# wangjie212/ManiSDP-matlab

Hardware: AMD Instinct MI355X
Metric: tCG Hess-vec prods/sec (n,p), G81 MaxCut (higher is better)
Workload: dtype f64; 1 GPU; Gset G81 MaxCut, ManiSDP_onlyunitdiag RTR call, n=20000, p=32; n=20000, p=32, nnz_C=92644, TR_maxiter=40, TR_maxinner=100, parallelism=rows1

## Files before the change

manisdp-matlab_amd/csrc/msdp_pipe.h:

```cpp
#pragma once
#include <type_traits>
#include "msdp_psync.h"

template <class F>
__device__ __forceinline__ bool psync8(unsigned long long* slots, unsigned gen, int G, double (&v)[8], double* sh8, double* shb8, int* err,
                                       int bid, int backoff, unsigned long long* tr, F on_ready) {
    const int lane = threadIdx.x & 63, w = threadIdx.x >> 6;
    {
        const bool h8 = (lane & 8) != 0;
        double a[4], b[2], x;
#pragma unroll
        for (int k = 0; k < 4; ++k) a[k] = msdp_swap_add<32>(v[k], v[4 + k]);
#pragma unroll
        for (int k = 0; k < 2; ++k) b[k] = msdp_swap_add<16>(a[k], a[2 + k]);
        x = (h8 ? b[1] : b[0]) + msdp_dpp<0x128>(h8 ? b[0] : b[1]);
        x += msdp_dpp<MSDP_DPP_XOR1>(x); x += msdp_dpp<MSDP_DPP_XOR2>(x); x += msdp_dpp<MSDP_DPP_HALF_MIRROR>(x);
        if ((lane & 7) == 0) sh8[(lane >> 3) * PWAVES + w] = x;
    }
    if (tr && threadIdx.x == 0) tr[4] = __builtin_readcyclecounter();
    asm volatile("s_waitcnt vmcnt(0)" ::: "memory");
    __syncthreads();
    if (tr && threadIdx.x == 0) tr[2] = __builtin_readcyclecounter();
    {
        unsigned long long* gbase = slots + (size_t)(gen % PSYNC_GEN) * PSYNC_REP * PSYNC_NV * MSDP_MAX_GRID;
        if (w == 0) {
            const int rep = lane / PSYNC_NV, vi = lane % PSYNC_NV;
            double s = 0.0;
            for (int i = 0; i < PWAVES; ++i) s += sh8[vi * PWAVES + i];
            asm volatile("s_waitcnt vmcnt(0)" ::: "memory");
            __hip_atomic_store(gbase + ((size_t)rep * PSYNC_NV + vi) * MSDP_MAX_GRID + bid,
                               (unsigned long long)__double_as_longlong(s), __ATOMIC_RELAXED, __HIP_MEMORY_SCOPE_AGENT);
        }
        const unsigned long long* p0 = gbase + ((size_t)(bid & (PSYNC_REP - 1)) * PSYNC_NV + w) * MSDP_MAX_GRID + lane;
        double r0;
        int spins = 0;
        bool fail = false;
        const int first = ((backoff >> 16) & 0xff) ? ((backoff >> 16) & 0xff) : 27;
        for (int q = 0; q < first; ++q) __builtin_amdgcn_s_sleep(1);
        if (tr && threadIdx.x == 0) tr[3] = __builtin_readcyclecounter();
        for (;;) {
            unsigned long long b0[4];
            asm volatile(
                "global_load_dwordx2 %0, %4, off sc1\n\t"
                "global_load_dwordx2 %1, %4, off offset:512 sc1\n\t"
                "global_load_dwordx2 %2, %4, off offset:1024 sc1\n\t"
                "global_load_dwordx2 %3, %4, off offset:1536 sc1\n\t"
                "s_waitcnt vmcnt(0)"
                : "=&v"(b0[0]), "=&v"(b0[1]), "=&v"(b0[2]), "=&v"(b0[3])
                : "v"(p0)
                : "memory");
            bool ok = true;
            double t0 = 0.0;
#pragma unroll
            for (int q = 0; q < 4; ++q) {
                if (lane + 64 * q < G) {
                    ok = ok && b0[q] != PSYNC_SENT;
                    t0 += __longlong_as_double((long long)b0[q]);
                }
            }
            r0 = t0;
            if (__builtin_amdgcn_ballot_w64(!ok) == 0ULL) break;
            ++spins;
            if (spins > PSYNC_SPIN_LIMIT ||
                ((spins & 1023) == 0 && __hip_atomic_load(err, __ATOMIC_RELAXED, __HIP_MEMORY_SCOPE_AGENT))) { fail = true; break; }
            for (int q = 0; q < ((backoff >> 8) & 0xff); ++q) __builtin_amdgcn_s_sleep(1);
        }
        if (tr && threadIdx.x == 0) tr[7] = (__builtin_readcyclecounter() << 4) + (unsigned long long)(spins < 15 ? spins : 15);
        if (!fail) on_ready();
        r0 = msdp_wave_sum(r0);
        if (lane == 0) {
            shb8[w] = r0; shb8[8 + w] = fail ? 1.0 : 0.0;
            if (fail) __hip_atomic_store(err, 1, __ATOMIC_RELAXED, __HIP_MEMORY_SCOPE_AGENT);
        }
        if (w == 0)
            __hip_atomic_store(slots + (size_t)((gen + PSYNC_GEN - 1) % PSYNC_GEN) * PSYNC_REP * PSYNC_NV * MSDP_MAX_GRID +
                                   (size_t)lane * MSDP_MAX_GRID + bid,
                               PSYNC_SENT, __ATOMIC_RELAXED, __HIP_MEMORY_SCOPE_AGENT);
    }
    asm volatile("s_waitcnt lgkmcnt(0)\n\ts_barrier" ::: "memory");
    double bad = 0.0;
#pragma unroll
    for (int i = 0; i < 8; ++i) { v[i] = msdp_readlane(shb8[i], 0); bad += msdp_readlane(shb8[8 + i], 0); }
    return bad == 0.0;
}

typedef unsigned long long v2ul __attribute__((ext_vector_type(2)));
template <class F>
__device__ __forceinline__ bool psync8_lines(unsigned long long* slots, unsigned gen, int G, double (&v)[8], double* sh8, double* shp, double* shb8,
                                             int* err, int bid, int backoff, unsigned long long* tr, F on_ready) {
    const int lane = threadIdx.x & 63, w = threadIdx.x >> 6;
    {
        const bool h8 = (lane & 8) != 0;
        double a[4], b[2], x;
#pragma unroll
        for (int k = 0; k < 4; ++k) a[k] = msdp_swap_add<32>(v[k], v[4 + k]);
#pragma unroll
        for (int k = 0; k < 2; ++k) b[k] = msdp_swap_add<16>(a[k], a[2 + k]);
        x = (h8 ? b[1] : b[0]) + msdp_dpp_all<0x128>(h8 ? b[0] : b[1]);
        x += msdp_dpp_all<MSDP_DPP_XOR1>(x); x += msdp_dpp_all<MSDP_DPP_XOR2>(x); x += msdp_dpp_all<MSDP_DPP_HALF_MIRROR>(x);
        if ((lane & 7) == 0) sh8[(lane >> 3) * PWAVES + w] = x;
    }
    if (tr && threadIdx.x == 0) tr[4] = __builtin_readcyclecounter();
    asm volatile("s_waitcnt vmcnt(0)" ::: "memory");
    __syncthreads();
    if (tr && threadIdx.x == 0) tr[2] = __builtin_readcyclecounter();
    unsigned long long* gbase = slots + (size_t)(gen % PSYNC_GEN) * PSYNC_REP * PSYNC_NV * MSDP_MAX_GRID;
    if (w == 0) {
        const int rep = lane >> 3, vi = lane & 7;
        double s = 0.0;
        for (int i = 0; i < PWAVES; ++i) s += sh8[vi * PWAVES + i];
        asm volatile("s_waitcnt vmcnt(0)" ::: "memory");
        __hip_atomic_store(gbase + (size_t)rep * PSYNC_NV * MSDP_MAX_GRID + (size_t)bid * 8 + vi,
                           (unsigned long long)__double_as_longlong(s), __ATOMIC_RELAXED, __HIP_MEMORY_SCOPE_AGENT);
    }
    const unsigned long long* p0 = gbase + (size_t)(bid & (PSYNC_REP - 1)) * PSYNC_NV * MSDP_MAX_GRID + (size_t)(32 * w + (lane >> 2)) * 8 + 2 * (lane & 3);
    const bool in0 = 32 * w + (lane >> 2) < G, in1 = 32 * w + 16 + (lane >> 2) < G;
    double t0 = 0.0, t1 = 0.0;
    int spins = 0;
    bool fail = false;
    const int first = ((backoff >> 16) & 0xff) ? ((backoff >> 16) & 0xff) : (backoff & 0xff);
    for (int q = 0; q < first; ++q) __builtin_amdgcn_s_sleep(1);
    if (tr && threadIdx.x == 0) tr[3] = __builtin_readcyclecounter();
    if (__builtin_amdgcn_ballot_w64(in0) != 0ULL) {
        for (;;) {
            v2ul a0, a1;
            asm volatile(
                "global_load_dwordx4 %0, %2, off sc1\n\t"
                "global_load_dwordx4 %1, %2, off offset:1024 sc1\n\t"
                "s_waitcnt vmcnt(0)"
                : "=&v"(a0), "=&v"(a1)
                : "v"(p0)
                : "memory");
            bool ok = true;
            t0 = 0.0; t1 = 0.0;
            if (in0) { ok = a0.x != PSYNC_SENT && a0.y != PSYNC_SENT; t0 = __longlong_as_double((long long)a0.x); t1 = __longlong_as_double((long long)a0.y); }
            if (in1) { ok = ok && a1.x != PSYNC_SENT && a1.y != PSYNC_SENT; t0 += __longlong_as_double((long long)a1.x); t1 += __longlong_as_double((long long)a1.y); }
            if (__builtin_amdgcn_ballot_w64(!ok) == 0ULL) break;
            ++spins;
            if (spins > PSYNC_SPIN_LIMIT ||
                ((spins & 1023) == 0 && __hip_atomic_load(err, __ATOMIC_RELAXED, __HIP_MEMORY_SCOPE_AGENT))) { fail = true; break; }
            for (int q = 0; q < ((backoff >> 8) & 0xff); ++q) __builtin_amdgcn_s_sleep(1);
        }
    }
    if (tr && threadIdx.x == 0) tr[7] = (__builtin_readcyclecounter() << 4) + (unsigned long long)(spins < 15 ? spins : 15);
    t0 += msdp_dpp_all<0x124>(t0); t1 += msdp_dpp_all<0x124>(t1);
    t0 += msdp_dpp_all<0x128>(t0); t1 += msdp_dpp_all<0x128>(t1);
    t0 = msdp_rowpair_sum<16>(t0); t1 = msdp_rowpair_sum<16>(t1);
    t0 = msdp_rowpair_sum<32>(t0); t1 = msdp_rowpair_sum<32>(t1);
    if (lane < 4) { shp[w * 8 + 2 * lane] = t0; shp[w * 8 + 2 * lane + 1] = t1; }
    if (lane == 0) {
        shb8[8 + w] = fail ? 1.0 : 0.0;
        if (fail) __hip_atomic_store(err, 1, __ATOMIC_RELAXED, __HIP_MEMORY_SCOPE_AGENT);
    }
    asm volatile("s_waitcnt lgkmcnt(0)\n\ts_barrier" ::: "memory");
    on_ready();
    if (w == 0)
        __hip_atomic_store(slots + (size_t)((gen + PSYNC_GEN - 1) % PSYNC_GEN) * PSYNC_REP * PSYNC_NV * MSDP_MAX_GRID +
                               (size_t)(lane >> 3) * PSYNC_NV * MSDP_MAX_GRID + (size_t)bid * 8 + (lane & 7),
                           PSYNC_SENT, __ATOMIC_RELAXED, __HIP_MEMORY_SCOPE_AGENT);
    double s = 0.0;
#pragma unroll
    for (int k = 0; k < PWAVES; ++k) s += shp[k * 8 + (lane & 7)];
    const double fl = shb8[8 + (lane & 7)];
#pragma unroll
    for (int i = 0; i < 8; ++i) v[i] = msdp_readlane(s, i);
    return __builtin_amdgcn_ballot_w64(fl != 0.0) == 0ULL;
}

__device__ __forceinline__ bool pbar8_lines(unsigned long long* slots, unsigned gen, int G, double* shb8, int* err, int bid, int backoff) {
    const int lane = threadIdx.x & 63, w = threadIdx.x >> 6;
    asm volatile("s_waitcnt vmcnt(0)" ::: "memory");
    __syncthreads();
    unsigned long long* gbase = slots + (size_t)(gen % PSYNC_GEN) * PSYNC_REP * PSYNC_NV * MSDP_MAX_GRID;
    if (w == 0) {
        asm volatile("s_waitcnt vmcnt(0)" ::: "memory");
        __hip_atomic_store(gbase + (size_t)(lane >> 3) * PSYNC_NV * MSDP_MAX_GRID + (size_t)bid * 8 + (lane & 7), 0ULL, __ATOMIC_RELAXED, __HIP_MEMORY_SCOPE_AGENT);
    }
    const unsigned long long* p0 = gbase + (size_t)(bid & (PSYNC_REP - 1)) * PSYNC_NV * MSDP_MAX_GRID + (size_t)(32 * w + (lane >> 2)) * 8 + 2 * (lane & 3);
    const bool in0 = 32 * w + (lane >> 2) < G, in1 = 32 * w + 16 + (lane >> 2) < G;
    int spins = 0;
    bool fail = false;
    const int first = ((backoff >> 16) & 0xff) ? ((backoff >> 16) & 0xff) : (backoff & 0xff);
    for (int q = 0; q < first; ++q) __builtin_amdgcn_s_sleep(1);
    if (__builtin_amdgcn_ballot_w64(in0) != 0ULL) {
        for (;;) {
            v2ul a0, a1;
            asm volatile(
                "global_load_dwordx4 %0, %2, off sc1\n\t"
                "global_load_dwordx4 %1, %2, off offset:1024 sc1\n\t"
                "s_waitcnt vmcnt(0)"
                : "=&v"(a0), "=&v"(a1)
                : "v"(p0)
                : "memory");
            bool ok = true;
            if (in0) ok = a0.x != PSYNC_SENT && a0.y != PSYNC_SENT;
            if (in1) ok = ok && a1.x != PSYNC_SENT && a1.y != PSYNC_SENT;
            if (__builtin_amdgcn_ballot_w64(!ok) == 0ULL) break;
            ++spins;
            if (spins > PSYNC_SPIN_LIMIT ||
                ((spins & 1023) == 0 && __hip_atomic_load(err, __ATOMIC_RELAXED, __HIP_MEMORY_SCOPE_AGENT))) { fail = true; break; }
            for (int q = 0; q < ((backoff >> 8) & 0xff); ++q) __builtin_amdgcn_s_sleep(1);
        }
    }
    if (lane == 0) {
        shb8[8 + w] = fail ? 1.0 : 0.0;
        if (fail) __hip_atomic_store(err, 1, __ATOMIC_RELAXED, __HIP_MEMORY_SCOPE_AGENT);
    }
    asm volatile("s_waitcnt lgkmcnt(0)\n\ts_barrier" ::: "memory");
    if (w == 0)
        __hip_atomic_store(slots + (size_t)((gen + PSYNC_GEN - 1) % PSYNC_GEN) * PSYNC_REP * PSYNC_NV * MSDP_MAX_GRID +
                               (size_t)(lane >> 3) * PSYNC_NV * MSDP_MAX_GRID + (size_t)bid * 8 + (lane & 7),
                           PSYNC_SENT, __ATOMIC_RELAXED, __HIP_MEMORY_SCOPE_AGENT);
    const double fl = shb8[8 + (lane & 7)];
    return __builtin_amdgcn_ballot_w64(fl != 0.0) == 0ULL;
}

template <class F>
__device__ __forceinline__ bool psync2_8(unsigned long long* blk, unsigned long long* const* peers, int N, int me, int ri, unsigned gen, int G,
                                         double (&v)[8], double* sh8, double* shb8, int* err, int bid, int backoff, F on_ready) {
    const int lane = threadIdx.x & 63, w = threadIdx.x >> 6;
    {
        const bool h8 = (lane & 8) != 0;
        double a[4], b[2], x;
#pragma unroll
        for (int k = 0; k < 4; ++k) a[k] = msdp_swap_add<32>(v[k], v[4 + k]);
#pragma unroll
        for (int k = 0; k < 2; ++k) b[k] = msdp_swap_add<16>(a[k], a[2 + k]);
        x = (h8 ? b[1] : b[0]) + msdp_dpp<0x128>(h8 ? b[0] : b[1]);
        x += msdp_dpp<MSDP_DPP_XOR1>(x); x += msdp_dpp<MSDP_DPP_XOR2>(x); x += msdp_dpp<MSDP_DPP_HALF_MIRROR>(x);
        if ((lane & 7) == 0) sh8[(lane >> 3) * PWAVES + w] = x;
    }
    asm volatile("s_waitcnt vmcnt(0)" ::: "memory");
    __syncthreads();
    unsigned long long* ls = blk + (size_t)ri * XR2_REGION;
    unsigned long long* ml = ls + PSYNC_REGION;
    unsigned long long* gbase = ls + (size_t)(gen % PSYNC_GEN) * PSYNC_REP * PSYNC_NV * MSDP_MAX_GRID;
    if (w == 0 && lane < 8) {
        double s = 0.0;
        for (int i = 0; i < PWAVES; ++i) s += sh8[lane * PWAVES + i];
        asm volatile("s_waitcnt vmcnt(0)" ::: "memory");
        __hip_atomic_store(gbase + (size_t)lane * MSDP_MAX_GRID + bid, (unsigned long long)__double_as_longlong(s), __ATOMIC_RELAXED, __HIP_MEMORY_SCOPE_AGENT);
    }
    bool fail = false;
    if (bid == 0) {
        const unsigned long long* p0 = gbase + (size_t)w * MSDP_MAX_GRID + lane;
        double r0 = 0.0;
        int spins = 0;
        for (;;) {
            unsigned long long b0[4];
            asm volatile(
                "global_load_dwordx2 %0, %4, off sc1\n\t"
                "global_load_dwordx2 %1, %4, off offset:512 sc1\n\t"
                "global_load_dwordx2 %2, %4, off offset:1024 sc1\n\t"
                "global_load_dwordx2 %3, %4, off offset:1536 sc1\n\t"
                "s_waitcnt vmcnt(0)"
                : "=&v"(b0[0]), "=&v"(b0[1]), "=&v"(b0[2]), "=&v"(b0[3])
                : "v"(p0)
                : "memory");
            bool ok = true;
            double t0 = 0.0;
#pragma unroll
            for (int q = 0; q < 4; ++q) {
                if (lane + 64 * q < G) {
                    ok = ok && b0[q] != PSYNC_SENT;
                    t0 += __longlong_as_double((long long)b0[q]);
                }
            }
            r0 = t0;
            if (__builtin_amdgcn_ballot_w64(!ok) == 0ULL) break;
            ++spins;
            if (spins > PSYNC_SPIN_LIMIT || ((spins & 1023) == 0 && __hip_atomic_load(err, __ATOMIC_RELAXED, __HIP_MEMORY_SCOPE_AGENT))) { fail = true; break; }
        }
        r0 = msdp_wave_sum(r0);
        if (!fail && lane < N)
            __hip_atomic_store(peers[lane] + (size_t)ri * XR2_REGION + PSYNC_REGION + ((size_t)(gen % PSYNC_GEN) * 8 + me) * 8 + w,
                               (unsigned long long)__double_as_longlong(r0), __ATOMIC_RELAXED, __HIP_MEMORY_SCOPE_SYSTEM);
        if (fail) xr2_fail(blk, peers, N, err);
        if (w > 0 && lane == 0) shb8[8 + w] = fail ? 1.0 : 0.0;
    }
    if (w == 0) {
        const unsigned long long* p = ml + (size_t)(gen % PSYNC_GEN) * 64 + lane;
        const bool need = (lane >> 3) < N;
        const int first = bid == 0 ? 0 : (((backoff >> 16) & 0xff) ? ((backoff >> 16) & 0xff) : (backoff & 0xff));
        for (int q = 0; q < first; ++q) __builtin_amdgcn_s_sleep(1);
        unsigned long long x = 0ULL;
        int spins = 0;
        for (;;) {
            x = ld_u64_sys(p);
            if (__builtin_amdgcn_ballot_w64(need && x == PSYNC_SENT) == 0ULL) break;
            ++spins;
            if (spins > PSYNC_SPIN_LIMIT || ((spins & 1023) == 0 && __hip_atomic_load(err, __ATOMIC_RELAXED, __HIP_MEMORY_SCOPE_AGENT))) { fail = true; break; }
            for (int q = 0; q < ((backoff >> 8) & 0xff); ++q) __builtin_amdgcn_s_sleep(1);
        }
        double t = need ? __longlong_as_double((long long)x) : 0.0;
        t += msdp_dpp<0x128>(t);
        t = msdp_rowpair_sum<16>(t);
        t = msdp_rowpair_sum<32>(t);
        if (lane < 8) { shb8[lane] = t; if (bid != 0 && lane > 0) shb8[8 + lane] = 0.0; }
        if (lane == 0) shb8[8] = fail ? 1.0 : 0.0;
        if (fail) xr2_fail(blk, peers, N, err);
        if (lane < PSYNC_NV)
            __hip_atomic_store(ls + (size_t)((gen + PSYNC_GEN - 1) % PSYNC_GEN) * PSYNC_REP * PSYNC_NV * MSDP_MAX_GRID + (size_t)lane * MSDP_MAX_GRID + bid,
                               PSYNC_SENT, __ATOMIC_RELAXED, __HIP_MEMORY_SCOPE_AGENT);
        if (bid == 0)
            __hip_atomic_store(ml + (size_t)((gen + PSYNC_GEN - 1) % PSYNC_GEN) * 64 + lane, PSYNC_SENT, __ATOMIC_RELAXED, __HIP_MEMORY_SCOPE_AGENT);
    }
    __syncthreads();
    on_ready();
    double bad = 0.0;
#pragma unroll
    for (int i = 0; i < 8; ++i) { v[i] = msdp_readlane(shb8[i], 0); bad += msdp_readlane(shb8[8 + i], 0); }
    return bad == 0.0;
}

#ifndef MSDP_PIPE_LINES
#define MSDP_PIPE_LINES 1
#endif
#if MSDP_PIPE_LINES
#define PSYNC8(slots, gen, G, v, sh8, shb8, err, bid, backoff, tr, f) psync8_lines(slots, gen, G, v, sh8, shp, shb8, err, bid, backoff, tr, f)
#else
#define PSYNC8(slots, gen, G, v, sh8, shb8, err, bid, backoff, tr, f) psync8(slots, gen, G, v, sh8, shb8, err, bid, backoff, tr, f)
#endif
template <int LPR, int EW, int R, bool TRACE, bool FUSE, int XRM = 0, int EP = 1>
__device__ __forceinline__ void tcg_pipe_body(const Dev& d, unsigned long long* slots, int* err, const int bx) {
    constexpr bool XR = XRM != 0, XTWO = XRM == 2;
    constexpr bool CSR = EW == 0;
    static_assert(!XR || (!FUSE && !TRACE), "cross-rank instances: per-iteration launches");
    static_assert(R <= 5, "pipelined trip: every vector in registers");
    static_assert(CSR ? (EP == 64 / LPR && !XR && !TRACE) : EP == 1, "CSR rows: one row per wave, one rank");
    static_assert(PSYNC_NV == 8 && PSYNC_REP * PSYNC_NV == 64, "psync8 posts one slot per lane of wave 0");
    constexpr bool BOFF = !(EW == 8 && LPR == 16), ROWB_INV = !XTWO, UMASK = !(FUSE && LPR == 16);
    extern __shared__ double lds[];
    __shared__ double sh8[8 * PWAVES];
    __shared__ double shp[8 * PWAVES];
    __shared__ double shb8[16];
    constexpr int RPW = 64 / (LPR * EP);
    constexpr int RSTEP = PWAVES * RPW;
    constexpr int ROWS = R * RSTEP;
    double2* Ys = reinterpret_cast<double2*>(lds);
    double2* Gs = Ys + R * PB;
    double* eGs = reinterpret_cast<double*>(Gs + R * PB);
    double* vs = eGs + ROWS;
    int* cs = reinterpret_cast<int*>(vs + EW * ROWS);
    int* ls = cs + EW * ROWS;
    double2* HQs = reinterpret_cast<double2*>(ls + EW * ROWS);
    unsigned long long* pds = reinterpret_cast<unsigned long long*>(HQs + 2 * R * PB);
    double2* YPs = HQs + 2 * R * PB;
    double2* GPs = YPs + R * PB;
    double* EGPs = reinterpret_cast<double*>(GPs + R * PB);

    const Ctl* c = d.ctl;
    const bool lead = bx == 0 && threadIdx.x == 0;
    const int k_tr = c->k;
    if (c->done) {
        if (lead) {
            frame_store(&d.F[0], c->gg, c->gg, 0.0, 0.0, 0.0, sqrt(c->gg), 0.0, 0.0, 0, 0, 5, 0, 0, 1);
            d.ctl->tcg_running = 0;
            msdp_publish(d, k_tr, 0, 0);
        }
        return;
    }
    if (lead && !FUSE) msdp_publish(d, k_tr, 0, 1);
    const int bid = (XR && !XTWO) ? d.xr_gid0 + bx : bx;
    const int GS = (XR && !XTWO) ? d.xr_gtot : d.G;
    const int xri = k_tr & 1;
    __shared__ unsigned long long* shpeer[XTWO ? 8 : 1];
    if (XTWO) {
        if (threadIdx.x < 8) shpeer[threadIdx.x] = threadIdx.x < d.xr2_n ? d.xr2_peers[threadIdx.x] : d.xr2_blk;
        psync2_reset_other(d.xr2_blk, xri ^ 1, bid, GS);
        asm volatile("s_waitcnt vmcnt(0)" ::: "memory");
    } else if (XR) {
        unsigned long long* other = slots + (size_t)(xri ^ 1) * PSYNC_REGION;
        slots += (size_t)xri * PSYNC_REGION;
        psync_reset_other(other, bid, GS);
        asm volatile("s_waitcnt vmcnt(0)" ::: "memory");
    } else if (!FUSE) psync_reset_other(slots + PSYNC_REGION, bid, GS);
    int lo, hi;
    msdp_chunk_rows(d.n_loc, d.G, lo, hi, 0, bx);
    const int lane = threadIdx.x & 63, wave = threadIdx.x >> 6;
    const int sub = lane & (LPR - 1), rsub = lane / (LPR * EP);
    const int epi = (lane / LPR) & (EP - 1);
    const bool colok_g = 2 * sub < d.ld;
    const bool colok = colok_g && epi == 0;
    int cur = c->cur;
    const bool bench = c->bench_mode != 0;
    double Delta = c->Delta;
    const double kappa = c->kappa, theta = c->theta;
    const int mininner = c->mininner, maxinner = c->maxinner;
    double gg = c->gg;
    double fx = c->fx;
    int k_it = c->k;
    const double Delta_bar = c->Delta_bar, rho_prime = c->rho_prime, rho_reg_opt = c->rho_reg, tolgradnorm = c->tolgradnorm;
    const int maxiter = c->maxiter;
    int n_acc = c->accepted, n_rej = c->rejected, n_hv = c->hessvecs, n_ce = c->cost_evals;
    const double* __restrict__ Yl = cur ? d.Y[1] : d.Y[0];
    const double* __restrict__ gl = cur ? d.Gr[1] : d.Gr[0];
    const double* __restrict__ eGl = cur ? d.eG[1] : d.eG[0];
    const int slot0 = wave * RPW + rsub;
#define SLOT(r) ((r) * RSTEP + slot0)
#define ROW(r) (lo + SLOT(r))
#define ROK(r) (ROW(r) < hi)
#define OK(r) (ROK(r) && colok)
    const unsigned rowb0 = ((unsigned)(lo + slot0) * (unsigned)d.ld + 2u * (unsigned)sub) * 8u;
#define ROWB(r) (ROWB_INV ? (rowb0 + (unsigned)((r) * RSTEP) * (unsigned)d.ld * 8u) : (((unsigned)ROW(r) * gld + 2 * sub) * 8u))
    const int refresh = c->pipe_refresh;
    const int backoff = (c->psync_backoff & 0xff00ffff) | ((((c->psync_backoff >> 16) & 0xff) ? ((c->psync_backoff >> 16) & 0xff) : (c->psync8_backoff & 0xff)) << 16);
    const double2 zz = make_double2(0.0, 0.0);
    const unsigned gld = (unsigned)d.ld;
    constexpr bool LOC = !CSR && R * EW <= 15;
    constexpr bool MULTI = LOC && !(FUSE && LPR >= 16);
    double2 eta[R], rr[R], md[R], hmd[R], cmd[R], ctr[R];
#pragma unroll
    for (int r = 0; r < R; ++r) {
        const bool rok = ROK(r);
        const int rc = rok ? ROW(r) : lo;
        const int64_t o = (int64_t)rc * d.ld + (colok ? 2 * sub : 0);
        double2 y = ld2(Yl + o), g = ld2(gl + o);
        if (!OK(r)) { y = zz; g = zz; }
        Ys[r * PB + threadIdx.x] = y; Gs[r * PB + threadIdx.x] = g;
        eta[r] = zz; rr[r] = g; md[r] = g; hmd[r] = zz; cmd[r] = zz; ctr[r] = zz;
    }
#pragma unroll 1
    for (int r = 0; r < (CSR ? 0 : R); ++r) {
        const bool rok = ROK(r);
        const int rc = rok ? ROW(r) : lo;
        const double egv = eGl[rc];
        int cw[EW > 0 ? EW : 1];
        double vw[EW > 0 ? EW : 1];
#pragma unroll
        for (int w = 0; w < EW; ++w) {
            cw[w] = XR ? d.xr_ellc[(int64_t)w * d.ell_stride + rc] : d.ellc[(int64_t)w * d.ell_stride + rc];
            vw[w] = d.ellv[(int64_t)w * d.ell_stride + rc];
        }
        int kw[EW > 0 ? EW : 1];
#pragma unroll
        for (int w = 0; w < EW; ++w) {
            if (!rok) vw[w] = 0.0;
            kw[w] = vw[w] == 0.0 ? 3 : (cw[w] == rc ? 0 : ((cw[w] >= lo && cw[w] < hi) ? 1 : 2));
        }
#pragma unroll
        for (int a = 0; a < (LOC ? EW - 1 : 0); ++a)
#pragma unroll
            for (int b2 = 0; b2 < EW - 1 - a; ++b2)
                if (kw[b2] > kw[b2 + 1]) {
                    const int tk = kw[b2]; kw[b2] = kw[b2 + 1]; kw[b2 + 1] = tk;
                    const int tc = cw[b2]; cw[b2] = cw[b2 + 1]; cw[b2 + 1] = tc;
                    const double tv = vw[b2]; vw[b2] = vw[b2 + 1]; vw[b2 + 1] = tv;
                }
        if (XR && sub == 0) {
#pragma unroll
            for (int t = 0; t < 2; ++t)
                pds[t * ROWS + SLOT(r)] = rok ? d.xr_paddr[(int64_t)t * d.n_loc + rc] : 0ULL;
        }
        if (sub == 0) {
            eGs[SLOT(r)] = rok ? egv : 0.0;
#pragma unroll
            for (int w = 0; w < EW; ++w) {
                cs[w * ROWS + SLOT(r)] = BOFF ? (int)((unsigned)cw[w] * gld * 8u) : cw[w];
                vs[w * ROWS + SLOT(r)] = vw[w];
                const int li = cw[w] - lo;
                const int el = (li / RSTEP) * PB + (li % RSTEP) * LPR;
                ls[w * ROWS + SLOT(r)] = kw[w] == 2 ? -1 : (kw[w] == 3 ? (2 << 24) : ((kw[w] == 0 ? (1 << 24) : 0) | el));
            }
        }
    }
    if (CSR) {
#pragma unroll
        for (int r = 0; r < R; ++r)
            if (sub == 0 && epi == 0) eGs[SLOT(r)] = ROK(r) ? eGl[ROW(r)] : 0.0;
    }
    __syncthreads();
    int nl = 0;
    if (LOC && c->pipe_local != 0) {
        bool lead_ok = true;
#pragma unroll
        for (int w = 0; w < EW; ++w) {
            bool glob = false;
#pragma unroll
            for (int r = 0; r < R; ++r) glob = glob || ls[w * ROWS + SLOT(r)] < 0;
            lead_ok = lead_ok && __builtin_amdgcn_ballot_w64(glob) == 0ULL;
            if (lead_ok) nl = w + 1;
        }
    }
    unsigned gen = 0;
    const unsigned half_bytes = XR ? (unsigned)(((size_t)d.xr_cap + (size_t)d.xr_halo) * d.ld * sizeof(double)) : (unsigned)((size_t)d.n_loc * d.ld * sizeof(double));
    const __amdgpu_buffer_rsrc_t rs_md = XR ? __builtin_amdgcn_make_buffer_rsrc(d.xr_rows[0], 0, 4u * half_bytes, 0x00020000)
                                            : __builtin_amdgcn_make_buffer_rsrc(d.mdx, 0, (FUSE ? 7u : 4u) * half_bytes, 0x00020000);
    bool xr_has_push = false, xr_has_push2 = false;
    if (XR) {
        bool any = false, any2 = false;
#pragma unroll
        for (int r = 0; r < R; ++r) { any = any || pds[SLOT(r)] != 0ULL; any2 = any2 || pds[ROWS + SLOT(r)] != 0ULL; }
        xr_has_push2 = __builtin_amdgcn_ballot_w64(any2) != 0ULL;
        xr_has_push = xr_has_push2 || __builtin_amdgcn_ballot_w64(any) != 0ULL;
    }
    auto xr_push = [&](int r, unsigned reg, double2 val) {
        if (!XR || !xr_has_push) return;
#pragma unroll
        for (int t = 0; t < 2; ++t) {
            if (t == 1 && !xr_has_push2) continue;
            const unsigned long long a = pds[t * ROWS + SLOT(r)];
            if (a != 0ULL && OK(r)) {
                double* ptr = reinterpret_cast<double*>(a + (unsigned long long)reg * half_bytes) + 2 * sub;
                if (XTWO) {
                    __hip_atomic_store(ptr, val.x, __ATOMIC_RELAXED, __HIP_MEMORY_SCOPE_SYSTEM);
                    __hip_atomic_store(ptr + 1, val.y, __ATOMIC_RELAXED, __HIP_MEMORY_SCOPE_SYSTEM);
                } else {
                    __hip_atomic_store(ptr, val.x, __ATOMIC_RELAXED, __HIP_MEMORY_SCOPE_AGENT);
                    __hip_atomic_store(ptr + 1, val.y, __ATOMIC_RELAXED, __HIP_MEMORY_SCOPE_AGENT);
                }
            }
        }
    };
    __amdgpu_buffer_rsrc_t rs_g = __builtin_amdgcn_make_buffer_rsrc(cur ? d.Gr[1] : d.Gr[0], 0, half_bytes, 0x00020000);
    unsigned g_base = 0u;
    const unsigned gcol = colok ? 2 * sub : 0, gcol8 = gcol * 8u;
    const bool idle_lanes = d.ld < 2 * LPR;
    constexpr int CSR_CB = 8;
    constexpr bool CSR_KEEP = CSR && R <= 2 && !FUSE;
    int ckeep[CSR_KEEP ? R : 1][CSR_CB];
    double vkeep[CSR_KEEP ? R : 1][CSR_CB];
    if (CSR_KEEP) {
#pragma unroll
        for (int r = 0; r < R; ++r) {
            const bool rok = ROK(r);
            const int s0 = rok ? d.rowptr[ROW(r)] : 0, s1 = rok ? d.rowptr[ROW(r) + 1] : 0;
#pragma unroll
            for (int u = 0; u < CSR_CB; ++u) {
                const int k = s0 + epi + u * EP;
                const bool in = k < s1;
                ckeep[r][u] = in ? d.colind[k] : (rok ? ROW(r) : lo);
                vkeep[r][u] = in ? d.cval[k] : 0.0;
            }
        }
    }
    auto csr_gather = [&](int r, __amdgpu_buffer_rsrc_t rs, unsigned base) -> double2 {
        constexpr int CB = CSR_CB;
        double2 acc = make_double2(0.0, 0.0);
        const bool rok = ROK(r);
        const int s0 = (CSR && rok) ? d.rowptr[ROW(r)] : 0, s1 = (CSR && rok) ? d.rowptr[ROW(r) + 1] : 0;
        const unsigned gcg = colok_g ? 2 * sub : 0;
        int kfirst = s0 + epi;
        if (CSR_KEEP) {
            double2 x[CB];
#pragma unroll
            for (int u = 0; u < CB; ++u) x[u] = ld2_sc1(rs, base + ((unsigned)ckeep[CSR_KEEP ? r : 0][u] * gld + gcg) * 8u);
#pragma unroll
            for (int u = 0; u < CB; ++u) { const double cv = vkeep[CSR_KEEP ? r : 0][u]; acc.x = fma(cv, x[u].x, acc.x); acc.y = fma(cv, x[u].y, acc.y); }
            kfirst += CB * EP;
        }
        for (int k0 = kfirst; __builtin_amdgcn_ballot_w64(k0 < s1) != 0ULL; k0 += CB * EP) {
            double2 x[CB];
            double cvk[CB];
#pragma unroll
            for (int u = 0; u < CB; ++u) {
                const int k = k0 + u * EP;
                const bool in = k < s1;
                const int cidx = in ? d.colind[k] : (rok ? ROW(r) : lo);
                cvk[u] = in ? d.cval[k] : 0.0;
                x[u] = ld2_sc1(rs, base + ((unsigned)cidx * gld + gcg) * 8u);
            }
#pragma unroll
            for (int u = 0; u < CB; ++u) { acc.x = fma(cvk[u], x[u].x, acc.x); acc.y = fma(cvk[u], x[u].y, acc.y); }
        }
#pragma unroll
        for (int m = LPR; m < LPR * EP; m <<= 1) { acc.x += __shfl_xor(acc.x, m); acc.y += __shfl_xor(acc.y, m); }
        if (!colok) acc = make_double2(0.0, 0.0);
        return acc;
    };

    double z_r = gg, d_Pd = gg, e_Pd = 0.0, e_Pe = 0.0, model_value = 0.0, alpha = 0.0, beta = 0.0;
    double norm_r0 = sqrt(gg);
    int j = 0, stop = 5;
    const int k_it0 = c->k;
#define FSTAMP(ph) do { if (TRACE && FUSE && threadIdx.x == 0 && k_it - k_it0 < MSDP_TRACE_NJ) \
        d.trace[((size_t)bx * MSDP_TRACE_NJ + (k_it - k_it0)) * 8 + (ph)] = __builtin_readcyclecounter(); } while (0)
    bool first = true, direct = false, failed = false;
    unsigned xq = 0;
    bool have_x = false;
#define MSDP_TRACE_KSEL 7
#define FTRIP_ON (TRACE && FUSE && k_it - k_it0 == MSDP_TRACE_KSEL && j < MSDP_TRACE_NJ)
#define FTRIP_PTR (d.trace + (size_t)GS * MSDP_TRACE_NJ * 8 + ((size_t)bx * MSDP_TRACE_NJ + j) * 8)
#define PTSTAMP(ph) do { if (!FUSE) { TSTAMP(ph); } else if (FTRIP_ON && threadIdx.x == 0) FTRIP_PTR[ph] = __builtin_readcyclecounter(); } while (0)
  auto trips = [&](auto nlc) {
    constexpr int NL = decltype(nlc)::value;
    constexpr int NG = EW - NL;
#ifndef MSDP_PIPE_VARIANT
#define MSDP_PIPE_VARIANT 0
#endif
    constexpr bool PREF = !CSR && R * NG <= ((FUSE && MSDP_PIPE_VARIANT == 0) ? 9 : 15);
    constexpr bool SPLIT = (MSDP_PIPE_VARIANT == 2 && FUSE) ? true : !PREF;
    double2 X[R][NG > 0 ? NG : 1];
    for (;;) {
        PTSTAMP(0);
#define PIPE_ISSUE(rs, base, w0) do { \
            _Pragma("unroll") for (int r = 0; r < R; ++r) \
            _Pragma("unroll") for (int w = 0; w < NG; ++w) { \
                if ((w0) + w < EW) { \
                    const unsigned coff = (unsigned)cs[((w0) + w) * ROWS + SLOT(r)]; \
                    X[r][w] = ld2_cp<XTWO ? 17 : MSDP_CPOL_SC1>((rs), (base) + (BOFF ? coff + gcol8 : (coff * gld + gcol) * 8u)); } } } while (0)
#define PIPE_FOLDX(r, acc, w0) do { \
            _Pragma("unroll") for (int w = 0; w < NG; ++w) { \
                if ((w0) + w < EW) { \
                    const double vv = vs[((w0) + w) * ROWS + SLOT(r)]; \
                    (acc).x = fma(vv, X[r][w].x, (acc).x); (acc).y = fma(vv, X[r][w].y, (acc).y); } } } while (0)
#define PIPE_FOLDL(r, acc, src) do { \
            _Pragma("unroll") for (int w = 0; w < NL; ++w) { \
                const double vv = vs[w * ROWS + SLOT(r)]; \
                const double2 xx = (src)[(ls[w * ROWS + SLOT(r)] & 0xffffff) + sub]; \
                (acc).x = fma(vv, xx.x, (acc).x); (acc).y = fma(vv, xx.y, (acc).y); } } while (0)
#define PIPE_GATHER_ALL(rs, base, dst) do { \
            if (CSR) { _Pragma("unroll") for (int r = 0; r < R; ++r) (dst)[r] = csr_gather(r, (rs), (base)); break; } \
            _Pragma("unroll") for (int r = 0; r < R; ++r) (dst)[r] = zz; \
            _Pragma("unroll") for (int w0 = 0; w0 < EW; w0 += (NG > 0 ? NG : 1)) { \
                PIPE_ISSUE(rs, base, w0); \
                _Pragma("unroll") for (int r = 0; r < R; ++r) PIPE_FOLDX(r, (dst)[r], w0); } \
            if (!colok) { _Pragma("unroll") for (int r = 0; r < R; ++r) (dst)[r] = zz; } } while (0)
        double v[8] = {0.0, 0.0, 0.0, 0.0, 0.0, 0.0, 0.0, 0.0};
        auto pre_sums = [&]() {
            if (!SPLIT) return;
#pragma unroll
            for (int r = 0; r < R; ++r) {
                const double2 g = Gs[r * PB + threadIdx.x], mdr = md[r], e0 = eta[r], rv = rr[r];
                const double2 rg = make_double2(rv.x - g.x, rv.y - g.y);
                v[3] += mdr.x * g.x + mdr.y * g.y;
                v[5] += mdr.x * rg.x + mdr.y * rg.y;
                v[6] += rv.x * rv.x + rv.y * rv.y;
                v[7] += (e0.x * g.x + e0.y * g.y) + 0.5 * (e0.x * rg.x + e0.y * rg.y);
            }
        };
        if (first) {
            pre_sums();
            PIPE_GATHER_ALL(rs_g, g_base, cmd);
#pragma unroll
            for (int r = 0; r < R; ++r) ctr[r] = cmd[r];
        } else {
            if (direct) {
                PIPE_GATHER_ALL(rs_md, 3u * half_bytes, ctr);
                PIPE_GATHER_ALL(rs_md, 2u * half_bytes, cmd);
            }
            if (!CSR && !have_x) PIPE_ISSUE(rs_md, (xq ^ 1u) * half_bytes, NL);
            pre_sums();
            auto products = [&](auto masked) {
#pragma unroll
                for (int r = 0; r < R; ++r) {
                    double2 a = zz;
                    if (CSR) a = csr_gather(r, rs_md, (xq ^ 1u) * half_bytes);
                    else { PIPE_FOLDL(r, a, HQs + (xq ^ 1u) * R * PB); PIPE_FOLDX(r, a, NL); }
                    if (decltype(masked)::value && !colok) a = zz;
                    ctr[r].x = fma(-alpha, a.x, ctr[r].x); ctr[r].y = fma(-alpha, a.y, ctr[r].y);
                    cmd[r].x = fma(beta, cmd[r].x, ctr[r].x); cmd[r].y = fma(beta, cmd[r].y, ctr[r].y);
                }
            };
            if (UMASK) { if (!CSR && idle_lanes) products(std::true_type()); else products(std::false_type()); } else products(std::true_type());
        }
        have_x = false;
        const bool pub = !first && refresh > 0 && ((j + 1) % refresh) == 0;
#pragma unroll
        for (int r = 0; r < R; ++r) {
            const double2 acc = cmd[r];
            const double2 y = Ys[r * PB + threadIdx.x], mdr = md[r], rv = rr[r];
            const double dot = msdp_group_sum_all<LPR>(acc.x * y.x + acc.y * y.y);
            const double eg = eGs[SLOT(r)];
            double2 hq = make_double2(acc.x - y.x * dot - mdr.x * eg, acc.y - y.y * dot - mdr.y * eg);
            if (!UMASK && !OK(r)) hq = zz;
            hmd[r] = hq;
            if (MULTI) HQs[xq * R * PB + r * PB + threadIdx.x] = hq;
            if (OK(r)) st2_sc1(rs_md, xq * half_bytes + ROWB(r), hq);
            xr_push(r, xq, hq);
            if (pub) {
                const double dn = msdp_group_sum_all<LPR>(rv.x * y.x + rv.y * y.y);
                if (OK(r)) {
                    st2_sc1(rs_md, 2u * half_bytes + ROWB(r), mdr);
                    st2_sc1(rs_md, 3u * half_bytes + ROWB(r), make_double2(rv.x - y.x * dn, rv.y - y.y * dn));
                }
                xr_push(r, 2u, mdr);
                xr_push(r, 3u, make_double2(rv.x - y.x * dn, rv.y - y.y * dn));
            }
            if (!SPLIT) {
                const double2 g = Gs[r * PB + threadIdx.x], e0 = eta[r];
                const double2 rg = make_double2(rv.x - g.x, rv.y - g.y);
                v[0] += mdr.x * hq.x + mdr.y * hq.y;
                v[1] += rv.x * hq.x + rv.y * hq.y;
                v[2] += hq.x * hq.x + hq.y * hq.y;
                v[3] += mdr.x * g.x + mdr.y * g.y;
                v[4] += e0.x * hq.x + e0.y * hq.y;
                v[5] += mdr.x * rg.x + mdr.y * rg.y;
                v[6] += rv.x * rv.x + rv.y * rv.y;
                v[7] += (e0.x * g.x + e0.y * g.y) + 0.5 * (e0.x * rg.x + e0.y * rg.y);
            }
        }
        if (SPLIT) {
#pragma unroll
            for (int r = 0; r < R; ++r) {
                const double2 hq = hmd[r], mdr = md[r], e0 = eta[r], rv = rr[r];
                v[0] += mdr.x * hq.x + mdr.y * hq.y;
                v[1] += rv.x * hq.x + rv.y * hq.y;
                v[2] += hq.x * hq.x + hq.y * hq.y;
                v[4] += e0.x * hq.x + e0.y * hq.y;
            }
        }
        PTSTAMP(1);
        if (TRACE && FUSE && j == 0) { FSTAMP(1); }
        auto next_gather = [&]() { if (PREF && !pub) { PIPE_ISSUE(rs_md, xq * half_bytes, NL); have_x = true; } };
        if (XTWO) {
            if (!psync2_8(d.xr2_blk, shpeer, d.xr2_n, d.xr2_me, xri, gen++, GS + d.xr2_skip, v, sh8, shb8, err, bid, backoff, next_gather)) { failed = true; break; }
        } else
        if (!PSYNC8(slots, gen++, GS, v, sh8, shb8, err, bid, backoff,
                    (TRACE && !FUSE && j >= MSDP_TRACE_J0 && j < MSDP_TRACE_J0 + MSDP_TRACE_NJ) ? d.trace + ((size_t)bx * MSDP_TRACE_NJ + (j - MSDP_TRACE_J0)) * 8 :
                    (FTRIP_ON ? FTRIP_PTR : nullptr),
                    next_gather)) { failed = true; break; }
        PTSTAMP(5);
        const double d_Hd = v[0];
        z_r = v[6];
        model_value = v[7];
        alpha = z_r / d_Hd;
        const double e_Pe_new = e_Pe + 2.0 * alpha * e_Pd + alpha * alpha * d_Pd;
        if (!bench && (d_Hd <= 0.0 || e_Pe_new >= Delta * Delta)) {
            const double tau = (-e_Pd + sqrt(e_Pd * e_Pd + d_Pd * (Delta * Delta - e_Pe))) / d_Pd;
#pragma unroll
            for (int r = 0; r < R; ++r) {
                eta[r].x -= tau * md[r].x; eta[r].y -= tau * md[r].y;
                rr[r].x -= tau * hmd[r].x; rr[r].y -= tau * hmd[r].y;
            }
            stop = (d_Hd <= 0.0) ? 1 : 2;
            ++j;
            break;
        }
        const double new_model = model_value - alpha * v[3] - 0.5 * alpha * (v[4] + v[5]) + 0.5 * alpha * alpha * d_Hd;
        const double r_r = fmax(z_r - 2.0 * alpha * v[1] + alpha * alpha * v[2], 0.0);
        e_Pe = e_Pe_new;
        if (!bench && new_model >= model_value) { stop = 6; ++j; break; }
#pragma unroll
        for (int r = 0; r < R; ++r) {
            eta[r].x -= alpha * md[r].x; eta[r].y -= alpha * md[r].y;
            rr[r].x -= alpha * hmd[r].x; rr[r].y -= alpha * hmd[r].y;
        }
        model_value = new_model;
        ++j;
        const double norm_r = sqrt(r_r);
        const double nr0t = (theta == 1.0) ? norm_r0 : pow(norm_r0, theta);
        if (!bench && j >= mininner && norm_r <= norm_r0 * fmin(nr0t, kappa)) {
            stop = (kappa < nr0t) ? 3 : 4;
            break;
        }
        if (j >= maxinner) break;
        beta = r_r / z_r;
        e_Pd = beta * (e_Pd + alpha * d_Pd);
        d_Pd = r_r + beta * beta * d_Pd;
        z_r = r_r;
#pragma unroll
        for (int r = 0; r < R; ++r) {
            const double2 y = Ys[r * PB + threadIdx.x];
            const double2 vv = make_double2(rr[r].x + beta * md[r].x, rr[r].y + beta * md[r].y);
            const double dot = msdp_group_sum_all<LPR>(vv.x * y.x + vv.y * y.y);
            md[r] = make_double2(vv.x - y.x * dot, vv.y - y.y * dot);
        }
        direct = pub;
        first = false;
        xq ^= 1u;
        { --j; PTSTAMP(6); ++j; }
    }
#undef PIPE_ISSUE
#undef PIPE_FOLDX
#undef PIPE_FOLDL
#undef PIPE_GATHER_ALL
#undef PTSTAMP
#undef FTRIP_ON
#undef FTRIP_PTR
  };
  if (XR && !XTWO && d.xr2_skip && bid == 0) return;
  if (XR) {
#pragma unroll
    for (int r = 0; r < R; ++r) {
        if (OK(r)) st2_sc1(rs_md, 2u * half_bytes + ROWB(r), md[r]);
        xr_push(r, 2u, md[r]);
    }
    asm volatile("s_waitcnt vmcnt(0)" ::: "memory");
    if (XTWO) {
        double z0 = 0.0, z1 = 0.0, z2 = 0.0;
        if (!psync2(d.xr2_blk, shpeer, d.xr2_n, d.xr2_me, xri, gen++, GS + d.xr2_skip, 0, z0, z1, z2, sh8, shb8, err, bid, backoff, false)) return;
    } else if (!pbar8_lines(slots, gen++, GS, shb8, err, bid, backoff)) return;
    rs_g = rs_md; g_base = 2u * half_bytes;
  }
  bool first_tr = true;
  for (;;) {
    FSTAMP(0);
    if (FUSE && !first_tr) {
#pragma unroll
        for (int r = 0; r < R; ++r) {
            const double2 g = Gs[r * PB + threadIdx.x];
            eta[r] = zz; rr[r] = g; md[r] = g; hmd[r] = zz; cmd[r] = zz; ctr[r] = zz;
        }
        z_r = gg; d_Pd = gg; e_Pd = 0.0; e_Pe = 0.0; model_value = 0.0; alpha = 0.0; beta = 0.0;
        norm_r0 = sqrt(gg);
        j = 0; stop = 5; first = true; direct = false; have_x = false;
    }
    first_tr = false;
    if (MULTI && nl >= 3) trips(std::integral_constant<int, MULTI ? 3 : 0>());
    else if (MULTI && nl == 2) trips(std::integral_constant<int, MULTI ? 2 : 0>());
    else trips(std::integral_constant<int, 0>());
    if (failed) return;
    if (TRACE && FUSE && threadIdx.x == 0 && k_it - k_it0 < MSDP_TRACE_NJ)
        d.trace[((size_t)bx * MSDP_TRACE_NJ + (k_it - k_it0)) * 8 + 2] = (__builtin_readcyclecounter() & 0x00ffffffffffffffULL) | ((unsigned long long)(j & 0xff) << 56);
    if (!FUSE) {
#pragma unroll
        for (int r = 0; r < R; ++r) {
            if (OK(r)) {
                const int64_t o = (int64_t)ROW(r) * d.ld + 2 * sub;
                const double2 g = Gs[r * PB + threadIdx.x];
                st2(d.eta[0] + o, eta[r]);
                st2(d.Heta[0] + o, make_double2(rr[r].x - g.x, rr[r].y - g.y));
            }
        }
        if (lead) {
            frame_store(&d.F[0], z_r, d_Pd, e_Pd, e_Pe, model_value, norm_r0, alpha, beta, 0, j, stop, 0, 0, 0);
            d.ctl->tcg_running = 0;
            msdp_publish(d, k_tr, j, 0);
        }
        return;
    }
    double tv[8] = {0.0, 0.0, 0.0, 0.0, 0.0, 0.0, 0.0, 0.0};
    const unsigned yx_base = 4u * half_bytes, gx_base = (5u + (unsigned)(cur ^ 1)) * half_bytes;
#pragma unroll
    for (int r = 0; r < R; ++r) {
        const double2 y = Ys[r * PB + threadIdx.x], g = Gs[r * PB + threadIdx.x];
        const double2 e0 = eta[r];
        const double2 he = make_double2(rr[r].x - g.x, rr[r].y - g.y);
        tv[2] += e0.x * (g.x + 0.5 * he.x) + e0.y * (g.y + 0.5 * he.y);
        const double2 x = make_double2(y.x + e0.x, y.y + e0.y);
        double nn = sqrt(msdp_group_sum_all<LPR>(x.x * x.x + x.y * x.y));
        if (!(nn > 0.0)) nn = 1.0;
        const double2 ypr = OK(r) ? make_double2(x.x / nn, x.y / nn) : zz;
        YPs[r * PB + threadIdx.x] = ypr;
        if (OK(r)) st2_sc1(rs_md, yx_base + ROWB(r), ypr);
    }
    FSTAMP(3);
    if (!pbar8_lines(slots, gen++, GS, shb8, err, bid, backoff)) return;
    FSTAMP(4);
    auto prop_finish = [&](int r, double2 acc) {
        if (!colok) acc = zz;
        const double2 ypr = YPs[r * PB + threadIdx.x];
        const double dot = msdp_group_sum_all<LPR>(acc.x * ypr.x + acc.y * ypr.y);
        const double2 gpr = OK(r) ? make_double2(acc.x - ypr.x * dot, acc.y - ypr.y * dot) : zz;
        GPs[r * PB + threadIdx.x] = gpr;
        tv[1] += gpr.x * gpr.x + gpr.y * gpr.y;
        if (sub == 0 && epi == 0) {
            EGPs[SLOT(r)] = ROK(r) ? dot : 0.0;
            if (ROK(r)) tv[0] += 0.5 * dot;
        }
        if (OK(r)) st2_sc1(rs_md, gx_base + ROWB(r), gpr);
    };
    if (CSR) {
#pragma unroll
        for (int r = 0; r < R; ++r) prop_finish(r, csr_gather(r, rs_md, yx_base));
    } else if (R * EW <= 16) {
        double2 XG[R][EW > 0 ? EW : 1];
#pragma unroll
        for (int r = 0; r < R; ++r)
#pragma unroll
            for (int w = 0; w < EW; ++w) XG[r][w] = ld2_sc1(rs_md, yx_base + (BOFF ? (unsigned)cs[w * ROWS + SLOT(r)] + gcol8 : ((unsigned)cs[w * ROWS + SLOT(r)] * gld + gcol) * 8u));
#pragma unroll
        for (int r = 0; r < R; ++r) {
            double2 acc = zz;
#pragma unroll
            for (int w = 0; w < EW; ++w) { const double vv = vs[w * ROWS + SLOT(r)]; acc.x = fma(vv, XG[r][w].x, acc.x); acc.y = fma(vv, XG[r][w].y, acc.y); }
            prop_finish(r, acc);
        }
    } else {
#pragma unroll 1
        for (int r = 0; r < R; ++r) {
            double2 xw[EW > 0 ? EW : 1];
#pragma unroll
            for (int w = 0; w < EW; ++w) xw[w] = ld2_sc1(rs_md, yx_base + (BOFF ? (unsigned)cs[w * ROWS + SLOT(r)] + gcol8 : ((unsigned)cs[w * ROWS + SLOT(r)] * gld + gcol) * 8u));
            double2 acc = zz;
#pragma unroll
            for (int w = 0; w < EW; ++w) { const double vv = vs[w * ROWS + SLOT(r)]; acc.x = fma(vv, xw[w].x, acc.x); acc.y = fma(vv, xw[w].y, acc.y); }
            prop_finish(r, acc);
        }
    }
    FSTAMP(5);
    if (!PSYNC8(slots, gen++, GS, tv, sh8, shb8, err, bid, backoff, nullptr, []() {})) return;
    FSTAMP(6);
    {
        const double fp = tv[0], ggp = tv[1], prd = tv[2];
        double rhonum = fx - fp;
        double rhoden = -prd;
        const double rreg = fmax(1.0, fabs(fx)) * 2.220446049250313e-16 * rho_reg_opt;
        rhonum += rreg;
        rhoden += rreg;
        const bool model_decreased = rhoden >= 0.0;
        const double rho = rhonum / rhoden;
        if (rho < 0.25 || !model_decreased || isnan(rho)) Delta = Delta / 4.0;
        else if (rho > 0.75 && (stop == 1 || stop == 2)) Delta = fmin(2.0 * Delta, Delta_bar);
        const bool accept = model_decreased && rho > rho_prime;
        if (accept) ++n_acc; else ++n_rej;
        n_hv += j;
        ++n_ce;
        if (lead) {
            Ctl* cw = d.ctl;
            cw->rho = rho; cw->rhonum = rhonum; cw->rhoden = rhoden; cw->fx_prop = fp; cw->gg_prop = ggp;
            cw->accepted = n_acc; cw->rejected = n_rej; cw->hessvecs = n_hv; cw->cost_evals = n_ce;
            cw->last_stop_inner = stop;
        }
        if (accept) {
            cur ^= 1;
            fx = fp; gg = ggp;
            { double2* t = Ys; Ys = YPs; YPs = t; }
            { double2* t = Gs; Gs = GPs; GPs = t; }
            { double* t = eGs; eGs = EGPs; EGPs = t; }
            rs_g = rs_md; g_base = gx_base;
        }
        FSTAMP(7);
        ++k_it;
    }
    if (sqrt(gg) < tolgradnorm || k_it >= maxiter) break;
  }
    {
        double* Yo = cur ? d.Y[1] : d.Y[0];
        double* Go = cur ? d.Gr[1] : d.Gr[0];
        double* eo = cur ? d.eG[1] : d.eG[0];
#pragma unroll
        for (int r = 0; r < R; ++r) {
            if (OK(r)) {
                const int64_t o = (int64_t)ROW(r) * d.ld + 2 * sub;
                st2(Yo + o, Ys[r * PB + threadIdx.x]);
                st2(Go + o, Gs[r * PB + threadIdx.x]);
            }
            if (sub == 0 && ROK(r)) eo[ROW(r)] = eGs[SLOT(r)];
        }
    }
    if (lead) {
        Ctl* cw = d.ctl;
        cw->fx = fx; cw->gg = gg; cw->norm_grad = sqrt(gg); cw->Delta = Delta;
        cw->k = k_it; cw->cur = cur;
        cw->done = 1;
        cw->tcg_running = 0;
        frame_store(&d.F[0], 0.0, 0.0, 0.0, 0.0, 0.0, 0.0, 0.0, 0.0, 0, 0, stop, 0, 0, 0);
    }
#undef FSTAMP
#undef SLOT
#undef ROW
#undef ROK
#undef OK
#undef ROWB
}

template <int LPR, int EW, int R, bool TRACE = false, bool FUSE = false, int XRM = 0, int EP = 1>
__global__ __launch_bounds__(PB) void k_tcg_pipe_obl(Dev d, unsigned long long* slots, int* err) {
    tcg_pipe_body<LPR, EW, R, TRACE, FUSE, XRM, EP>(d, slots, err, (int)blockIdx.x);
}
```

Measured before the change: 198,900 Hess-vec/s.

## Precompute row projection dots while waiting in grid psync to hide reductions

Adds an on_wait hook to the psync8 grid-reduction routines and uses it to compute three per-row group sums (r·y, Hd·y, d·y) while blocks spin waiting for peers. After the sync, the projection dot for the new direction is rebuilt algebraically from those sums using alpha and beta, which removes a group reduction from the critical path after each barrier. It also hoists the pow-based inner stopping threshold out of the inner loop. The cost is extra LDS storage and three reductions instead of one, plus a small change in floating-point rounding order.

```diff
diff --git a/manisdp-matlab_amd/csrc/msdp_pipe.h b/manisdp-matlab_amd/csrc/msdp_pipe.h
--- a/manisdp-matlab_amd/csrc/msdp_pipe.h
+++ b/manisdp-matlab_amd/csrc/msdp_pipe.h
@@ -2,9 +2,9 @@
 #include <type_traits>
 #include "msdp_psync.h"
 
-template <class F>
+template <class F, class W>
 __device__ __forceinline__ bool psync8(unsigned long long* slots, unsigned gen, int G, double (&v)[8], double* sh8, double* shb8, int* err,
-                                       int bid, int backoff, unsigned long long* tr, F on_ready) {
+                                       int bid, int backoff, unsigned long long* tr, F on_ready, W on_wait) {
     const int lane = threadIdx.x & 63, w = threadIdx.x >> 6;
     {
         const bool h8 = (lane & 8) != 0;
@@ -35,6 +35,7 @@
         double r0;
         int spins = 0;
         bool fail = false;
+        on_wait();
         const int first = ((backoff >> 16) & 0xff) ? ((backoff >> 16) & 0xff) : 27;
         for (int q = 0; q < first; ++q) __builtin_amdgcn_s_sleep(1);
         if (tr && threadIdx.x == 0) tr[3] = __builtin_readcyclecounter();
@@ -85,9 +86,9 @@
 }
 
 typedef unsigned long long v2ul __attribute__((ext_vector_type(2)));
-template <class F>
+template <class F, class W>
 __device__ __forceinline__ bool psync8_lines(unsigned long long* slots, unsigned gen, int G, double (&v)[8], double* sh8, double* shp, double* shb8,
-                                             int* err, int bid, int backoff, unsigned long long* tr, F on_ready) {
+                                             int* err, int bid, int backoff, unsigned long long* tr, F on_ready, W on_wait) {
     const int lane = threadIdx.x & 63, w = threadIdx.x >> 6;
     {
         const bool h8 = (lane & 8) != 0;
@@ -115,6 +116,7 @@
     }
     const unsigned long long* p0 = gbase + (size_t)(bid & (PSYNC_REP - 1)) * PSYNC_NV * MSDP_MAX_GRID + (size_t)(32 * w + (lane >> 2)) * 8 + 2 * (lane & 3);
     const bool in0 = 32 * w + (lane >> 2) < G, in1 = 32 * w + 16 + (lane >> 2) < G;
+    on_wait();
     double t0 = 0.0, t1 = 0.0;
     int spins = 0;
     bool fail = false;
@@ -317,9 +319,9 @@
 #define MSDP_PIPE_LINES 1
 #endif
 #if MSDP_PIPE_LINES
-#define PSYNC8(slots, gen, G, v, sh8, shb8, err, bid, backoff, tr, f) psync8_lines(slots, gen, G, v, sh8, shp, shb8, err, bid, backoff, tr, f)
+#define PSYNC8(slots, gen, G, v, sh8, shb8, err, bid, backoff, tr, f, fw) psync8_lines(slots, gen, G, v, sh8, shp, shb8, err, bid, backoff, tr, f, fw)
 #else
-#define PSYNC8(slots, gen, G, v, sh8, shb8, err, bid, backoff, tr, f) psync8(slots, gen, G, v, sh8, shb8, err, bid, backoff, tr, f)
+#define PSYNC8(slots, gen, G, v, sh8, shb8, err, bid, backoff, tr, f, fw) psync8(slots, gen, G, v, sh8, shb8, err, bid, backoff, tr, f, fw)
 #endif
 template <int LPR, int EW, int R, bool TRACE, bool FUSE, int XRM = 0, int EP = 1>
 __device__ __forceinline__ void tcg_pipe_body(const Dev& d, unsigned long long* slots, int* err, const int bx) {
@@ -330,6 +332,7 @@
     static_assert(CSR ? (EP == 64 / LPR && !XR && !TRACE) : EP == 1, "CSR rows: one row per wave, one rank");
     static_assert(PSYNC_NV == 8 && PSYNC_REP * PSYNC_NV == 64, "psync8 posts one slot per lane of wave 0");
     constexpr bool BOFF = !(EW == 8 && LPR == 16), ROWB_INV = !XTWO, UMASK = !(FUSE && LPR == 16);
+    constexpr bool EDOT = !XTWO;
     extern __shared__ double lds[];
     __shared__ double sh8[8 * PWAVES];
     __shared__ double shp[8 * PWAVES];
@@ -409,6 +412,8 @@
     const unsigned gld = (unsigned)d.ld;
     constexpr bool LOC = !CSR && R * EW <= 15;
     constexpr bool MULTI = LOC && !(FUSE && LPR >= 16);
+    __shared__ __attribute__((aligned(16))) double dts_own[(EDOT && MULTI) ? 4 * ROWS : 2];
+    double* const dts = MULTI ? dts_own : reinterpret_cast<double*>(HQs);
     double2 eta[R], rr[R], md[R], hmd[R], cmd[R], ctr[R];
 #pragma unroll
     for (int r = 0; r < R; ++r) {
@@ -571,6 +576,8 @@
 
     double z_r = gg, d_Pd = gg, e_Pd = 0.0, e_Pe = 0.0, model_value = 0.0, alpha = 0.0, beta = 0.0;
     double norm_r0 = sqrt(gg);
+    double nr0t = (theta == 1.0) ? norm_r0 : pow(norm_r0, theta);
+    double r_stop = norm_r0 * fmin(nr0t, kappa);
     int j = 0, stop = 5;
     const int k_it0 = c->k;
 #define FSTAMP(ph) do { if (TRACE && FUSE && threadIdx.x == 0 && k_it - k_it0 < MSDP_TRACE_NJ) \
@@ -703,13 +710,29 @@
         PTSTAMP(1);
         if (TRACE && FUSE && j == 0) { FSTAMP(1); }
         auto next_gather = [&]() { if (PREF && !pub) { PIPE_ISSUE(rs_md, xq * half_bytes, NL); have_x = true; } };
+        auto row_dots = [&]() {
+            if (!EDOT) return;
+            __builtin_amdgcn_sched_barrier(0);
+#pragma unroll
+            for (int r = 0; r < R; ++r) {
+                const double2 y = Ys[r * PB + threadIdx.x];
+                const double s1 = msdp_group_sum_all<LPR>(rr[r].x * y.x + rr[r].y * y.y);
+                const double s2 = msdp_group_sum_all<LPR>(hmd[r].x * y.x + hmd[r].y * y.y);
+                const double s3 = msdp_group_sum_all<LPR>(md[r].x * y.x + md[r].y * y.y);
+                if (sub == 0 && epi == 0) {
+                    *reinterpret_cast<double2*>(&dts[4 * SLOT(r)]) = make_double2(s1, s2);
+                    dts[4 * SLOT(r) + 2] = s3;
+                }
+            }
+            __builtin_amdgcn_sched_barrier(0);
+        };
         if (XTWO) {
             if (!psync2_8(d.xr2_blk, shpeer, d.xr2_n, d.xr2_me, xri, gen++, GS + d.xr2_skip, v, sh8, shb8, err, bid, backoff, next_gather)) { failed = true; break; }
         } else
         if (!PSYNC8(slots, gen++, GS, v, sh8, shb8, err, bid, backoff,
                     (TRACE && !FUSE && j >= MSDP_TRACE_J0 && j < MSDP_TRACE_J0 + MSDP_TRACE_NJ) ? d.trace + ((size_t)bx * MSDP_TRACE_NJ + (j - MSDP_TRACE_J0)) * 8 :
                     (FTRIP_ON ? FTRIP_PTR : nullptr),
-                    next_gather)) { failed = true; break; }
+                    next_gather, row_dots)) { failed = true; break; }
         PTSTAMP(5);
         const double d_Hd = v[0];
         z_r = v[6];
@@ -739,8 +762,7 @@
         model_value = new_model;
         ++j;
         const double norm_r = sqrt(r_r);
-        const double nr0t = (theta == 1.0) ? norm_r0 : pow(norm_r0, theta);
-        if (!bench && j >= mininner && norm_r <= norm_r0 * fmin(nr0t, kappa)) {
+        if (!bench && j >= mininner && norm_r <= r_stop) {
             stop = (kappa < nr0t) ? 3 : 4;
             break;
         }
@@ -753,7 +775,11 @@
         for (int r = 0; r < R; ++r) {
             const double2 y = Ys[r * PB + threadIdx.x];
             const double2 vv = make_double2(rr[r].x + beta * md[r].x, rr[r].y + beta * md[r].y);
-            const double dot = msdp_group_sum_all<LPR>(vv.x * y.x + vv.y * y.y);
+            double dot;
+            if (EDOT) {
+                const double2 s12 = *reinterpret_cast<const double2*>(&dts[4 * SLOT(r)]);
+                dot = fma(beta, dts[4 * SLOT(r) + 2], fma(-alpha, s12.y, s12.x));
+            } else dot = msdp_group_sum_all<LPR>(vv.x * y.x + vv.y * y.y);
             md[r] = make_double2(vv.x - y.x * dot, vv.y - y.y * dot);
         }
         direct = pub;
@@ -794,6 +820,8 @@
         }
         z_r = gg; d_Pd = gg; e_Pd = 0.0; e_Pe = 0.0; model_value = 0.0; alpha = 0.0; beta = 0.0;
         norm_r0 = sqrt(gg);
+        nr0t = (theta == 1.0) ? norm_r0 : pow(norm_r0, theta);
+        r_stop = norm_r0 * fmin(nr0t, kappa);
         j = 0; stop = 5; first = true; direct = false; have_x = false;
     }
     first_tr = false;
@@ -880,7 +908,7 @@
         }
     }
     FSTAMP(5);
-    if (!PSYNC8(slots, gen++, GS, tv, sh8, shb8, err, bid, backoff, nullptr, []() {})) return;
+    if (!PSYNC8(slots, gen++, GS, tv, sh8, shb8, err, bid, backoff, nullptr, []() {}, []() {})) return;
     FSTAMP(6);
     {
         const double fp = tv[0], ggp = tv[1], prd = tv[2];
```

Result: slower. 188,200 Hess-vec/s (-5.4%).
